# endernewton/tf-faster-rcnn

Hardware: AMD Instinct MI355X
Metric: images/sec (600×1000) ResNet-101 Faster R-CNN at 1/2/4/8 MI355X (higher is better)
Workload: dtype f32 (operands, accumulators, results; GEMMs with Cin, Cout % 128 == 0 form each f32 product from two-piece fp16 operands with an exact power-of-two scale per 128-k block on the fp16 matrix pipe -- 3 MFMAs / product, dropped terms <= 3 * 2^-22, measured error vs float64 below the f32-MFMA kernel's; o

## Files before the change

scratch/h2_conv3.py:

```python
import os, sys
ROOT = os.path.dirname(os.path.dirname(os.path.abspath(__file__)))
sys.path[:0] = [os.path.join(ROOT, "tf-faster-rcnn_amd")]
args = [a for a in sys.argv[1:]]
lib_path, single = None, 0
if "--lib" in args:
    i = args.index("--lib"); lib_path = args[i + 1]; del args[i:i + 2]
if "--single" in args:
    i = args.index("--single"); single = int(args[i + 1]); del args[i:i + 2]
import frcnn_hip
if lib_path:
    frcnn_hip.LIB_PATH = os.path.abspath(lib_path)
import numpy as np, torch
from frcnn_hip import ops
dev = torch.device("cuda:0")
shapes = {
    "b4c3x8":  (1, 117600, 2048, 512, True, True, True, 0),
    "b4c3x8m": (8, 14700, 2048, 512, True, False, False, 49),
    "b3c3x8":  (1, 19152, 1024, 256, True, True, True, 0),
    "b2c3x8":  (1, 75000, 512, 128, True, True, True, 0),
    "b4c3x8p": (1, 117600, 2048, 512, "planes", False, True, 0),
    "b3c3x8p": (1, 19152, 1024, 256, "planes", False, True, 0),
    "b3scx8":  (1, 19152, 1024, 512, False, True, True, 0),
    "w7x8":    (121, 2400, 512, 512, False, True, False, 0),
    "w3x8":    (36, 1280, 256, 256, False, True, False, 0),
    "wrpnx8":  (36, 1280, 512, 1024, False, True, False, 0),
    "b4c1x8":  (1, 117600, 512, 2048, False, False, True, 0),
    "b3c1x8":  (1, 19152, 256, 1024, False, True, False, 0),
    "cal_k128": (1, 117600, 128, 128, "planes", False, True, 0),
    "b4c3x1":  (1, 14700, 2048, 512, True, True, True, 0),
    "b3c3x1":  (1, 2394, 1024, 256, True, True, True, 0),
}
cfgs = [int(c) for c in (args[0] if args else "9,21,12").split(",")]
only = args[1].split(",") if len(args) > 1 else ["b4c3x8", "b4c3x8m", "b3c3x8", "b2c3x8", "w7x8", "w3x8", "b4c1x8", "b3c1x8"]
if not single:
    print("%-8s %-4s %9s %9s %8s %8s  %s" % ("shape", "cfg", "med_us", "min_us", "TFLOP/s", "GB/s", "bits vs cfg %d" % cfgs[0]))
for name in only:
    G, M, N, K, has_res, f32o, planes, mean_rows = shapes[name]
    torch.manual_seed(1)
    x = torch.randn(G * M, K, device=dev).clamp(min=0) * torch.exp(torch.rand(G * M, K, device=dev) * 4 - 2)
    shared_w = mean_rows > 0
    w = torch.randn(1 if shared_w else G, N, K, device=dev) * 0.05
    b = torch.randn(N, device=dev) if (G == 1 or shared_w) else None
    res = torch.randn(G * M, N, device=dev) if has_res else None
    if has_res == "planes":
        res = ops.h2_split(res.clamp(min=0))
    xp, wp = ops.h2_split(x), ops.h2_pack_w(w)
    del x
    outs, outp = {}, {}
    share = G * M * N * 4 > (1 << 29)
    for c in cfgs:
        if mean_rows:
            outs[c] = torch.empty(G * M // mean_rows, N, device=dev)
        else:
            outs[c] = (outs[cfgs[0]] if (share and c != cfgs[0]) else torch.empty(G * M, N, device=dev)) if f32o else None
            outp[c] = (outp[cfgs[0]] if (share and c != cfgs[0]) else ops.H2.empty(G * M, N, dev)) if planes else None

    def run(c):
        if mean_rows:
            return ops.gemm_h2_mean(xp, wp, G, M, N, K, b, res, 1, mean_rows, out=outs[c], cfg=c)
        return ops.gemm_h2(xp, wp, G, M, N, K, b, res, 1, out=outs[c], out_planes=outp.get(c), want_f32=f32o, cfg=c)

    if single:
        for _ in range(single):
            run(cfgs[0])
        torch.cuda.synchronize()
        break
    def digest(c):
        parts = []
        if outs.get(c) is not None:
            parts.append(outs[c].view(torch.int32).to(torch.int64).sum())
            parts.append((outs[c].view(torch.int32).to(torch.int64) * torch.arange(1, outs[c].numel() + 1, device=dev).view(outs[c].shape) % 1000003).sum())
        if outp.get(c) is not None:
            pv = outp[c].planes.view(torch.int16).to(torch.int64)
            parts.append(pv.sum()); parts.append((pv * (torch.arange(pv.numel(), device=dev) % 8191 + 1)).sum())
            parts.append(outp[c].inv.view(torch.int32).to(torch.int64).sum())
        return tuple(int(p) for p in parts)
    digs = {}
    for c in cfgs:
        if outs.get(c) is not None: outs[c].fill_(float("nan"))
        if outp.get(c) is not None: outp[c].planes.zero_(); outp[c].inv.zero_()
        try:
            run(c); torch.cuda.synchronize()
            digs[c] = digest(c)
        except Exception as e:
            digs[c] = "unsupported (%s)" % (str(e)[:60],)
    live = [c for c in cfgs if not isinstance(digs[c], str)]
    times = {c: [] for c in live}
    for r in range(6):
        for c in live:
            e0, e1 = torch.cuda.Event(enable_timing=True), torch.cuda.Event(enable_timing=True)
            e0.record()
            for _ in range(6): run(c)
            e1.record(); torch.cuda.synchronize()
            if r: times[c].append(e0.elapsed_time(e1) * 1000 / 6)
    nbytes = 4.0 * G * M * K + 4.0 * (w.numel()) + G * M * N * 4.0 * ((1 if has_res else 0) + (1 if f32o else 0) + (1 if planes else 0))
    for c in cfgs:
        if c not in live:
            print("%-8s %-4d %s" % (name, c, digs[c]), flush=True)
            continue
        med = float(np.median(times[c]))
        print("%-8s %-4d %9.1f %9.1f %8.1f %8.0f  %s" % (name, c, med, min(times[c]), 2.0 * G * M * N * K / med / 1e6, nbytes / med / 1e3,
                                                       "identical" if digs[c] == digs[cfgs[0]] else "DIFFERENT"), flush=True)
    del outs, outp, xp, res
    torch.cuda.empty_cache()
```

tf-faster-rcnn_amd/csrc/gemm_h2.hip:

```cpp
#include "h2_common.h"
#include <mutex>
#include <type_traits>

typedef float f32x16 __attribute__((ext_vector_type(16)));
typedef _Float16 h8 __attribute__((ext_vector_type(8)));

#define LDS_AS __attribute__((address_space(3)))

struct GemmH2Params {
  const unsigned short* x; const float* x_inv; const unsigned short* w; const float* w_inv;
  const float* bias; const float* res; const unsigned short* resp; const float* resp_inv; float* y; unsigned short* yp; float* y_inv;
  int M, N, K, batch, act, nsteps, mtiles, ntiles;
  long long Mtot;
  int wshare;
  const float* mask;
  float* mean_part; int mean_rows;
};

__device__ __forceinline__ void h2_glds16(unsigned voff, const void* sbase, unsigned lds_base) {
  unsigned keep;
  asm volatile(
      "s_mov_b32 %0, m0\n\t"
      "s_mov_b32 m0, %3\n\t"
      "s_nop 0\n\t"
      "global_load_lds_dwordx4 %1, %2\n\t"
      "s_mov_b32 m0, %0"
      : "=&s"(keep)
      : "v"(voff), "s"(sbase), "s"(lds_base)
      : "memory");
}

__device__ __forceinline__ void h2_glds4(unsigned voff, const void* sbase, unsigned lds_base) {
  unsigned keep;
  asm volatile(
      "s_mov_b32 %0, m0\n\t"
      "s_mov_b32 m0, %3\n\t"
      "s_nop 0\n\t"
      "global_load_lds_dword %1, %2\n\t"
      "s_mov_b32 m0, %0"
      : "=&s"(keep)
      : "v"(voff), "s"(sbase), "s"(lds_base)
      : "memory");
}

__device__ __forceinline__ void h2_glds16c(unsigned voff, const void* sbase, unsigned lds_base) {
  asm volatile(
      "s_mov_b32 m0, %2\n\t"
      "s_nop 0\n\t"
      "global_load_lds_dwordx4 %0, %1"
      :
      : "v"(voff), "s"(sbase), "s"(lds_base)
      : "memory");
}
__device__ __forceinline__ void h2_glds4c(unsigned voff, const void* sbase, unsigned lds_base) {
  asm volatile(
      "s_mov_b32 m0, %2\n\t"
      "s_nop 0\n\t"
      "global_load_lds_dword %0, %1"
      :
      : "v"(voff), "s"(sbase), "s"(lds_base)
      : "memory");
}

template <int N>
__device__ __forceinline__ void h2_wait_vmcnt() {
  asm volatile("s_waitcnt vmcnt(%0)" ::"n"(N) : "memory");
}

enum H2Tune : int {
  H2_SCALES_ONCE = 2,
  H2_PINGPONG = 32,
  H2_MASKED = 128,
  H2_LIGHT_BOUNDARY = 256,
  H2_STORE16 = 512,
  H2_DEFERRED = 1024,
#ifdef FRCNN_ABLATION
  H2_NO_MFMA = 2048,
  H2_NO_FRAG = 4096,
  H2_NO_LOAD = 8192,
#endif
};

template <int BM, int BN, int WM, int WN, int NS, int TUNE>
struct H2Lds {
  static constexpr int NW = (BM / WM) * (BN / WN);
  static constexpr bool PP = (TUNE & H2_PINGPONG) != 0;
  static constexpr int XP = BM * 64, WP = BN * 64;
  static constexpr int S_OFF = 2 * XP + 2 * WP;
  static constexpr int STAGE = S_OFF + (PP ? 0 : 1024);
  static constexpr int RED_OFF = NS * STAGE;
  static constexpr int S2_OFF = RED_OFF + (BN / WN) * BM * 4;
  static constexpr int CB_OFF = S2_OFF + (PP ? NW * 512 : (TUNE & H2_SCALES_ONCE) ? 2048 : 0);
  static constexpr int TOTAL = CB_OFF + ((TUNE & H2_LIGHT_BOUNDARY) ? 2 * 2 * BN * 4 : 0);
};

template <int BM, int BN, int WM, int WN, int NS, int WPE = 2, int TUNE = 0>
__global__ __launch_bounds__((BM / WM) * (BN / WN) * 64) __attribute__((amdgpu_waves_per_eu(WPE))) void k_gemm_h2(const GemmH2Params p) {
  constexpr int NW = (BM / WM) * (BN / WN);
  constexpr int TM = WM / 32, TN = WN / 32;
  constexpr int LA = 2 * BM / 16 / NW;
  constexpr int LB = 2 * BN / 16 / NW;
  constexpr int G = LA + LB;
  constexpr int SL = BM / 64;
  constexpr bool ONCE = (TUNE & H2_SCALES_ONCE) != 0;
  constexpr bool PP = (TUNE & H2_PINGPONG) != 0;
  constexpr bool MASKED = (TUNE & H2_MASKED) != 0;
  constexpr bool LTB = (TUNE & H2_LIGHT_BOUNDARY) != 0;
  constexpr bool W21 = (TUNE & H2_STORE16) != 0;
  constexpr bool DE = (TUNE & H2_DEFERRED) != 0;
  using L = H2Lds<BM, BN, WM, WN, NS, TUNE>;
  constexpr int XP = L::XP, WP = L::WP, S_OFF = L::S_OFF, STAGE = L::STAGE, RED_OFF = L::RED_OFF, S2_OFF = L::S2_OFF, CB_OFF = L::CB_OFF;
  static_assert(!LTB || (!PP && NS == 2 && NW >= 3 && BN % 64 == 0), "light boundary: the two-slot one-barrier-per-slab schedule");
  static_assert(!DE || (LTB && W21 && BN == H2_KB), "deferred epilogue: built on the light boundary's LDS constants and counted waits");
  static_assert(!PP || (NW == 8 && NS == 3 && ONCE && BM == 256 && WM == 64 && BN == 128 && WN == 64),
                "ping-pong geometry: 8 waves as 4 (M) x 2 (N), waves 0-3 = the upper half of the rows");
  static_assert((2 * BM / 16) % NW == 0 && (2 * BN / 16) % NW == 0, "tile/wave mismatch");
  static_assert(BM <= 256 && NS >= 2 && NS <= 4, "stage layout");
  static_assert((NS - 2) * (G + SL) <= 63, "vmcnt range");
  extern __shared__ __attribute__((aligned(16))) char smem[];

  const int tid = threadIdx.x, lane = tid & 63;
  const int wave = __builtin_amdgcn_readfirstlane(tid >> 6);
  const int per = p.mtiles * p.ntiles, T = per * p.batch;
  const int xcd = blockIdx.x & 7, wx = blockIdx.x >> 3, W8 = gridDim.x >> 3;
  const int tq = T / 8, tr = T % 8, tn = tq + (xcd < tr ? 1 : 0);
  const int t_end = (xcd < tr ? xcd * (tq + 1) : tr * (tq + 1) + (xcd - tr) * tq) + tn;
  const int tile0 = t_end - tn + wx;
  if (tile0 >= t_end) return;
  const int my_tiles = (t_end - tile0 + W8 - 1) / W8;
  int left = __builtin_amdgcn_readfirstlane(my_tiles * p.nsteps);

  const int wmi = wave / (BN / WN), wni = wave % (BN / WN);
  const int wm0 = wmi * WM, wn0 = wni * WN;
  const int frow = lane & 31, khalf = lane >> 5;

  const size_t xplane = (size_t)p.Mtot * p.K * 2, wplane = (size_t)p.N * p.K * 2;
  unsigned a_off[LA], b_off[LB], s_off[SL];
  const char* i_xb = nullptr; const char* i_wb = nullptr; const char* i_sb = nullptr;
  int i_tile = tile0, i_step = 0, i_par = 0, c_par = 0;
  int i_g = 0, i_bn0 = 0, i_cpar = 0, c_cpar = 0;
  int pend = 0;
#pragma unroll
  for (int t = 0; t < LB; ++t) {
    const int u = wave * LB + t, plane = u / (BN / 16), row = (u % (BN / 16)) * 16 + (lane >> 2), pos = lane & 3;
    b_off[t] = (unsigned)((size_t)plane * wplane + (size_t)row * p.K * 2 + ((pos ^ ((row >> 2) & 3)) * 16));
  }
  auto tile_coords = [&](int tl, int& g, int& mt, int& nt) {
    g = tl / per;
    const int rem = tl - g * per;
    mt = rem / p.ntiles;
    nt = rem - mt * p.ntiles;
  };
  auto set_tile = [&](int tl) {
    int g, mt, nt;
    tile_coords(tl, g, mt, nt);
    const int bm0 = mt * BM, bn0 = nt * BN;
    const size_t row0 = (size_t)g * p.M + bm0;
    i_g = g; i_bn0 = bn0;
    i_xb = (const char*)p.x + row0 * p.K * 2;
    i_wb = (const char*)p.w + ((size_t)(p.wshare ? 0 : g) * 2 * p.N + bn0) * p.K * 2;
    i_sb = (const char*)(p.x_inv + row0);
#pragma unroll
    for (int t = 0; t < LA; ++t) {
      const int u = wave * LA + t, plane = u / (BM / 16), row = (u % (BM / 16)) * 16 + (lane >> 2), pos = lane & 3;
      const int rr = min(row, p.M - 1 - bm0);
      a_off[t] = (unsigned)((size_t)plane * xplane + (size_t)rr * p.K * 2 + ((pos ^ ((row >> 2) & 3)) * 16));
    }
    const long long last = p.Mtot - 1 - (long long)row0;
#pragma unroll
    for (int j = 0; j < SL; ++j) s_off[j] = (unsigned)(min((long long)((PP ? wm0 : j * 64) + lane), last) * 4);
  };
  const unsigned lds0 = (unsigned)(size_t)(LDS_AS char*)smem;
  auto uniform_ptr = [](const char* q) {
    const unsigned long long v = (unsigned long long)q;
    const unsigned lo = __builtin_amdgcn_readfirstlane((unsigned)v), hi = __builtin_amdgcn_readfirstlane((unsigned)(v >> 32));
    return (const char*)(((unsigned long long)hi << 32) | lo);
  };
  auto issue_one = [&](int buf, int t) {
    const unsigned sb = lds0 + (unsigned)(buf * STAGE);
    if constexpr (PP) {
      if (t < LA) h2_glds16c(a_off[t], uniform_ptr(i_xb), __builtin_amdgcn_readfirstlane(sb + (wave * LA + t) * 1024));
      else if (t < G) h2_glds16c(b_off[t - LA], uniform_ptr(i_wb), __builtin_amdgcn_readfirstlane(sb + 2 * XP + (wave * LB + (t - LA)) * 1024));
      else if (t == G && (i_step & 3) == 0) {
        h2_glds4c(s_off[0], uniform_ptr(i_sb), __builtin_amdgcn_readfirstlane(lds0 + S2_OFF + (wave * 2 + i_par) * 256));
        i_par ^= 1;
      }
      return;
    }
    if (t < LA) h2_glds16(a_off[t], uniform_ptr(i_xb), __builtin_amdgcn_readfirstlane(sb + (wave * LA + t) * 1024));
    else if (t < G) h2_glds16(b_off[t - LA], uniform_ptr(i_wb), __builtin_amdgcn_readfirstlane(sb + 2 * XP + (wave * LB + (t - LA)) * 1024));
    else if (wave == 0) {
      const int j = t - G;
      if (!ONCE) h2_glds4(s_off[j], uniform_ptr(i_sb), __builtin_amdgcn_readfirstlane(sb + S_OFF + j * 256));
      else if ((i_step & 3) == 0) {
        h2_glds4(s_off[j], uniform_ptr(i_sb), __builtin_amdgcn_readfirstlane(lds0 + S2_OFF + i_par * 1024 + j * 256));
        if (j == SL - 1) i_par ^= 1;
      }
    }
  };
  static_assert(!ONCE || NS == 2 || PP, "scales-once needs the uncounted wait of the two-stage ring");
  auto issue_advance = [&]() {
    --left;
    if (++i_step == p.nsteps) {
      i_step = 0; i_tile += W8;
      if (left > 0) set_tile(i_tile);
    } else {
      i_xb += 64; i_wb += 64;
      if ((i_step & 3) == 0) i_sb += (size_t)p.Mtot * 4;
    }
  };

  auto issue_cb = [&]() {
    const unsigned cb = lds0 + CB_OFF + i_cpar * (2 * BN * 4);
    if (wave == 1) {
#pragma unroll
      for (int j = 0; j < BN / 64; ++j)
        h2_glds4((unsigned)(lane * 4), uniform_ptr((const char*)(p.w_inv + (size_t)(p.wshare ? 0 : i_g) * p.N + i_bn0 + j * 64)),
                 __builtin_amdgcn_readfirstlane(cb + j * 256));
    }
    if (wave == 2 && p.bias) {
#pragma unroll
      for (int j = 0; j < BN / 64; ++j)
        h2_glds4((unsigned)(lane * 4), uniform_ptr((const char*)(p.bias + i_bn0 + j * 64)), __builtin_amdgcn_readfirstlane(cb + BN * 4 + j * 256));
    }
    i_cpar ^= 1;
  };
  auto wait_pending = [&](int n) {
    if constexpr (DE) {
      if (n >= 32) {
        if (n >= 48) { if (n >= 56) h2_wait_vmcnt<56>(); else h2_wait_vmcnt<48>(); }
        else { if (n >= 40) h2_wait_vmcnt<40>(); else h2_wait_vmcnt<32>(); }
      } else {
        if (n >= 16) { if (n >= 24) h2_wait_vmcnt<24>(); else h2_wait_vmcnt<16>(); }
        else { if (n >= 8) h2_wait_vmcnt<8>(); else h2_wait_vmcnt<0>(); }
      }
      return;
    }
    if (n >= 63) h2_wait_vmcnt<63>();
    else if (n >= 48) h2_wait_vmcnt<48>();
    else if (n >= 32) h2_wait_vmcnt<32>();
    else if (n >= 16) h2_wait_vmcnt<16>();
    else h2_wait_vmcnt<0>();
  };

  f32x16 tot[TM][TN], tmp[TM][TN];
  const int sw = (frow >> 2) & 3;
  const int x_row = (wm0 + frow) * 64, w_row = 2 * XP + (wn0 + frow) * 64;

#ifdef FRCNN_ABLATION
  constexpr bool NO_MFMA = (TUNE & H2_NO_MFMA) != 0, NO_FRAG = (TUNE & H2_NO_FRAG) != 0, NO_LOAD = (TUNE & H2_NO_LOAD) != 0;
#else
  constexpr bool NO_MFMA = false, NO_FRAG = false, NO_LOAD = false;
#endif
  h8 kxh[NO_FRAG ? TM : 1], kxl[NO_FRAG ? TM : 1], kwh[NO_FRAG ? TN : 1], kwl[NO_FRAG ? TN : 1];
  (void)kxh; (void)kxl; (void)kwh; (void)kwl;
  auto slab_mfma = [&](int cur, auto first_c) {
    constexpr bool FIRST = decltype(first_c)::value;
    const char* sb = smem + cur * STAGE;
#pragma unroll
    for (int t = 0; t < 2; ++t) {
      h8 xh[TM], xl[TM], wh[TN], wl[TN];
      if constexpr (NO_FRAG) {
        if (FIRST && t == 0) {
#pragma unroll
          for (int j = 0; j < TN; ++j) {
            const char* q = sb + w_row + j * 32 * 64 + ((khalf ^ sw) * 16);
            kwh[j] = __builtin_bit_cast(h8, *(const uint4*)(q));
            kwl[j] = __builtin_bit_cast(h8, *(const uint4*)(q + WP));
          }
#pragma unroll
          for (int i = 0; i < TM; ++i) {
            const char* q = sb + x_row + i * 32 * 64 + ((khalf ^ sw) * 16);
            kxh[i] = __builtin_bit_cast(h8, *(const uint4*)(q));
            kxl[i] = __builtin_bit_cast(h8, *(const uint4*)(q + XP));
          }
        }
#pragma unroll
        for (int j = 0; j < TN; ++j) { wh[j] = kwh[j]; wl[j] = kwl[j]; asm volatile("" : "+v"(wh[j]), "+v"(wl[j])); }
#pragma unroll
        for (int i = 0; i < TM; ++i) { xh[i] = kxh[i]; xl[i] = kxl[i]; asm volatile("" : "+v"(xh[i]), "+v"(xl[i])); }
      } else {
#pragma unroll
      for (int j = 0; j < TN; ++j) {
        const char* q = sb + w_row + j * 32 * 64 + (((2 * t + khalf) ^ sw) * 16);
        wh[j] = __builtin_bit_cast(h8, *(const uint4*)(q));
        wl[j] = __builtin_bit_cast(h8, *(const uint4*)(q + WP));
      }
#pragma unroll
      for (int i = 0; i < TM; ++i) {
        const char* q = sb + x_row + i * 32 * 64 + (((2 * t + khalf) ^ sw) * 16);
        xh[i] = __builtin_bit_cast(h8, *(const uint4*)(q));
        xl[i] = __builtin_bit_cast(h8, *(const uint4*)(q + XP));
      }
      }
      if constexpr (NO_MFMA) {
#pragma unroll
        for (int j = 0; j < TN; ++j) asm volatile("" :: "v"(wh[j]), "v"(wl[j]));
#pragma unroll
        for (int i = 0; i < TM; ++i) asm volatile("" :: "v"(xh[i]), "v"(xl[i]));
        if (FIRST && t == 0) {
#pragma unroll
          for (int i = 0; i < TM; ++i)
#pragma unroll
            for (int j = 0; j < TN; ++j)
#pragma unroll
              for (int r = 0; r < 16; ++r) tmp[i][j][r] = 0.f;
        }
        continue;
      }
#pragma unroll
      for (int i = 0; i < TM; ++i)
#pragma unroll
        for (int j = 0; j < TN; ++j) {
          if (FIRST && t == 0) {
            f32x16 z;
#pragma unroll
            for (int r = 0; r < 16; ++r) z[r] = 0.f;
            tmp[i][j] = __builtin_amdgcn_mfma_f32_32x32x16_f16(wh[j], xh[i], z, 0, 0, 0);
          } else {
            tmp[i][j] = __builtin_amdgcn_mfma_f32_32x32x16_f16(wh[j], xh[i], tmp[i][j], 0, 0, 0);
          }
        }
#pragma unroll
      for (int i = 0; i < TM; ++i)
#pragma unroll
        for (int j = 0; j < TN; ++j) {
          tmp[i][j] = __builtin_amdgcn_mfma_f32_32x32x16_f16(wl[j], xh[i], tmp[i][j], 0, 0, 0);
        }
#pragma unroll
      for (int i = 0; i < TM; ++i)
#pragma unroll
        for (int j = 0; j < TN; ++j) {
          tmp[i][j] = __builtin_amdgcn_mfma_f32_32x32x16_f16(wh[j], xl[i], tmp[i][j], 0, 0, 0);
        }
    }
  };

  int c_tile = tile0, c_step = 0, cur = 0, nxt = 0;
  int c_bm0 = 0, c_bn0 = 0, c_g = 0;
  auto set_ctile = [&](int tl) {
    int g, mt, nt;
    tile_coords(tl, g, mt, nt);
    c_bm0 = mt * BM; c_bn0 = nt * BN; c_g = g;
  };
  const float act_lo = p.act == FRCNN_ACT_NONE ? -__builtin_inff() : 0.f;
  const float act_hi = p.act == FRCNN_ACT_RELU6 ? 6.f : __builtin_inff();

  auto rsrc_f = [&](const void* base, long long elems_left, int esize) {
    const long long bytes = elems_left * esize;
    return __builtin_amdgcn_make_buffer_rsrc((void*)base, 0, (int)max(0ll, min(bytes, 0x7fffffffll)), 0x00020000);
  };

  struct TileRef { int bm0, bn0, g, cpar; };
  auto ent_rsrc = [&](const void* base, int g, int esize) {
    const char* b = (const char*)base + (size_t)g * p.M * p.N * esize;
    return __builtin_amdgcn_make_buffer_rsrc((void*)b, 0, p.M * p.N * esize, 0x00020000);
  };
  const int lo4 = (frow * p.N + 4 * khalf) * 4;
  auto lo2_of = [&]() { int v = lo4; asm volatile("" : "+v"(v)); return v >> 1; };
  auto lo2w_of = [&]() { int v = lo4; asm volatile("" : "+v"(v)); return (v >> 1) + 8 * (int)(threadIdx.x >> 5 & 1); };
  auto sub_off = [&](const auto& T, int i, int j) {
    return __builtin_amdgcn_readfirstlane((T.bm0 + wm0 + i * 32) * p.N + T.bn0 + wn0 + j * 32);
  };

  float rri[TM];
  (void)rri;
  auto load_res_raw = [&](int i) {
    typedef unsigned u32x4 __attribute__((ext_vector_type(4)));
    const TileRef C{c_bm0, c_bn0, c_g, c_cpar};
    const bool planes = !p.res && p.resp;
    const auto none = __builtin_amdgcn_make_buffer_rsrc((void*)nullptr, 0, 0, 0x00020000);
    const auto r_even = p.res ? ent_rsrc(p.res, c_g, 4) : planes ? ent_rsrc(p.resp, c_g, 2) : none;
    const auto r_odd = p.res ? r_even : planes ? ent_rsrc(p.resp + (size_t)p.Mtot * p.N, c_g, 2) : none;
    const int step_q = planes ? 0 : 32, step_p = planes ? 32 : 0;
    int base = lo4;
    asm volatile("" : "+v"(base));
    if (planes) base = (base >> 1) + 8 * (int)(threadIdx.x >> 5 & 1);
#pragma unroll
    for (int j = 0; j < TN; ++j) {
      const int vo = base + sub_off(C, i, j) * (planes ? 2 : 4);
#pragma unroll
      for (int q = 0; q < 4; ++q) {
        const u32x4 ld = __builtin_amdgcn_raw_buffer_load_b128((q & 1) ? r_odd : r_even, vo, q * step_q + (q >> 1) * step_p, 0);
        tot[i][j][4 * q + 0] = __uint_as_float(ld[0]); tot[i][j][4 * q + 1] = __uint_as_float(ld[1]);
        tot[i][j][4 * q + 2] = __uint_as_float(ld[2]); tot[i][j][4 * q + 3] = __uint_as_float(ld[3]);
      }
      pend += 4;
    }
    if (p.resp) rri[i] = p.resp_inv[(size_t)(c_bn0 / H2_KB) * p.Mtot + (size_t)c_g * p.M + min(c_bm0 + wm0 + i * 32 + frow, p.M - 1)];
  };
  auto init_tot = [&]() {
    if constexpr (DE) return;
    const size_t row_base = (size_t)c_g * p.M;
    typedef unsigned u32x4 __attribute__((ext_vector_type(4)));
    if (p.res) {
#pragma unroll
      for (int i = 0; i < TM; ++i)
#pragma unroll
        for (int j = 0; j < TN; ++j) {
          const int m0 = c_bm0 + wm0 + i * 32, nc = c_bn0 + wn0 + j * 32;
          const auto rr = rsrc_f(p.res + (long long)(row_base + m0) * p.N + nc, (long long)(p.M - m0) * p.N - nc, 4);
#pragma unroll
          for (int q = 0; q < 4; ++q) {
            const u32x4 ld = __builtin_amdgcn_raw_buffer_load_b128(rr, (frow * p.N + 4 * khalf) * 4 + 32 * q, 0, 0);
            tot[i][j][4 * q + 0] = __uint_as_float(ld[0]); tot[i][j][4 * q + 1] = __uint_as_float(ld[1]);
            tot[i][j][4 * q + 2] = __uint_as_float(ld[2]); tot[i][j][4 * q + 3] = __uint_as_float(ld[3]);
          }
        }
      pend += TM * TN * 4;
    } else if (p.resp) {
      float ri[TM];
#pragma unroll
      for (int i = 0; i < TM; ++i)
        ri[i] = p.resp_inv[(size_t)(c_bn0 / H2_KB) * p.Mtot + row_base + min(c_bm0 + wm0 + i * 32 + frow, p.M - 1)];
      h4 hv[TM][TN][4], lv[TM][TN][4];
#pragma unroll
      for (int i = 0; i < TM; ++i)
#pragma unroll
        for (int j = 0; j < TN; ++j) {
          const int m0 = c_bm0 + wm0 + i * 32, nc = c_bn0 + wn0 + j * 32;
          const long long sbase = (long long)(row_base + m0) * p.N + nc, left_e = (long long)(p.M - m0) * p.N - nc;
          const auto rh = rsrc_f(p.resp + sbase, left_e, 2), rl = rsrc_f(p.resp + (size_t)p.Mtot * p.N + sbase, left_e, 2);
#pragma unroll
          for (int q = 0; q < 4; ++q) {
            const int lo2 = (frow * p.N + 4 * khalf) * 2 + 16 * q;
            hv[i][j][q] = __builtin_bit_cast(h4, __builtin_amdgcn_raw_buffer_load_b64(rh, lo2, 0, 0));
            lv[i][j][q] = __builtin_bit_cast(h4, __builtin_amdgcn_raw_buffer_load_b64(rl, lo2, 0, 0));
          }
        }
#pragma unroll
      for (int i = 0; i < TM; ++i)
#pragma unroll
        for (int j = 0; j < TN; ++j)
#pragma unroll
          for (int q = 0; q < 4; ++q)
#pragma unroll
            for (int e = 0; e < 4; ++e) tot[i][j][4 * q + e] = ((float)hv[i][j][q][e] + (float)lv[i][j][q][e]) * ri[i];
    } else {
#pragma unroll
      for (int i = 0; i < TM; ++i)
#pragma unroll
        for (int j = 0; j < TN; ++j)
#pragma unroll
          for (int r = 0; r < 16; ++r) tot[i][j][r] = 0.f;
    }
    if constexpr (LTB) return;
    float4 wi[TN][4], bv[TN][4];
#pragma unroll
    for (int j = 0; j < TN; ++j)
#pragma unroll
      for (int q = 0; q < 4; ++q)
        wi[j][q] = *(const float4*)(p.w_inv + (size_t)(p.wshare ? 0 : c_g) * p.N + c_bn0 + wn0 + j * 32 + 4 * khalf + 8 * q);
    if (p.bias) {
#pragma unroll
      for (int j = 0; j < TN; ++j)
#pragma unroll
        for (int q = 0; q < 4; ++q) bv[j][q] = *(const float4*)(p.bias + c_bn0 + wn0 + j * 32 + 4 * khalf + 8 * q);
    } else {
#pragma unroll
      for (int j = 0; j < TN; ++j)
#pragma unroll
        for (int q = 0; q < 4; ++q) bv[j][q] = make_float4(0.f, 0.f, 0.f, 0.f);
    }
#pragma unroll
    for (int j = 0; j < TN; ++j)
#pragma unroll
      for (int q = 0; q < 4; ++q) {
        const float s0 = __uint_as_float(0x7f000000u - __float_as_uint(wi[j][q].x)), s1 = __uint_as_float(0x7f000000u - __float_as_uint(wi[j][q].y));
        const float s2 = __uint_as_float(0x7f000000u - __float_as_uint(wi[j][q].z)), s3 = __uint_as_float(0x7f000000u - __float_as_uint(wi[j][q].w));
#pragma unroll
        for (int i = 0; i < TM; ++i) {
          tot[i][j][4 * q + 0] = (tot[i][j][4 * q + 0] + bv[j][q].x) * s0;
          tot[i][j][4 * q + 1] = (tot[i][j][4 * q + 1] + bv[j][q].y) * s1;
          tot[i][j][4 * q + 2] = (tot[i][j][4 * q + 2] + bv[j][q].z) * s2;
          tot[i][j][4 * q + 3] = (tot[i][j][4 * q + 3] + bv[j][q].w) * s3;
        }
      }
  };

  auto ep_scale_act = [&](const TileRef& T) {
#pragma unroll
    for (int j = 0; j < TN; ++j) {
      const int n0 = T.bn0 + wn0 + j * 32 + 4 * khalf;
#pragma unroll
      for (int q = 0; q < 4; ++q) {
        const float4 wi = LTB ? *(const float4*)(smem + CB_OFF + T.cpar * (2 * BN * 4) + (wn0 + j * 32 + 4 * khalf + 8 * q) * 4)
                             : *(const float4*)(p.w_inv + (size_t)(p.wshare ? 0 : T.g) * p.N + n0 + 8 * q);
#pragma unroll
        for (int i = 0; i < TM; ++i) {
          tot[i][j][4 * q + 0] = act_clamp(tot[i][j][4 * q + 0] * wi.x, act_lo, act_hi);
          tot[i][j][4 * q + 1] = act_clamp(tot[i][j][4 * q + 1] * wi.y, act_lo, act_hi);
          tot[i][j][4 * q + 2] = act_clamp(tot[i][j][4 * q + 2] * wi.z, act_lo, act_hi);
          tot[i][j][4 * q + 3] = act_clamp(tot[i][j][4 * q + 3] * wi.w, act_lo, act_hi);
        }
      }
    }
  };
  auto ep_mask = [&](const TileRef& T) {
    if (MASKED && p.mask) {
      const auto rk = ent_rsrc(p.mask, T.g, 4);
#pragma unroll
      for (int i = 0; i < TM; ++i)
#pragma unroll
        for (int j = 0; j < TN; ++j) {
          const int vo = lo4 + sub_off(T, i, j) * 4;
          typedef unsigned u32x4 __attribute__((ext_vector_type(4)));
          u32x4 k[4];
#pragma unroll
          for (int q = 0; q < 4; ++q) k[q] = __builtin_amdgcn_raw_buffer_load_b128(rk, vo + 32 * q, 0, 0);
#pragma unroll
          for (int q = 0; q < 4; ++q)
#pragma unroll
            for (int e = 0; e < 4; ++e) tot[i][j][4 * q + e] = __uint_as_float(k[q][e]) > 0.f ? tot[i][j][4 * q + e] : 0.f;
        }
      pend += TM * TN * 4;
    }
  };
  auto ep_mean = [&](const TileRef& T) {
    const int nblk = (p.M + 31) >> 5;
#pragma unroll
    for (int i = 0; i < TM; ++i) {
      const int mb = T.bm0 + wm0 + i * 32;
      if (mb >= p.M) continue;
      const int m = mb + frow, g0 = mb / p.mean_rows, gid = m / p.mean_rows;
      const bool in_a = m < p.M && gid == g0, in_b = m < p.M && gid == g0 + 1;
      float* dst = p.mean_part + ((size_t)T.g * nblk + (mb >> 5)) * 2 * p.N;
#pragma unroll
      for (int j = 0; j < TN; ++j) {
        const int n0 = T.bn0 + wn0 + j * 32 + 4 * khalf;
#pragma unroll
        for (int q = 0; q < 4; ++q) {
          float a[4], b[4];
#pragma unroll
          for (int e = 0; e < 4; ++e) {
            const float v = tot[i][j][4 * q + e];
            a[e] = in_a ? v : 0.f;
            b[e] = in_b ? v : 0.f;
          }
#pragma unroll
          for (int o = 1; o < 32; o <<= 1)
#pragma unroll
            for (int e = 0; e < 4; ++e) {
              a[e] += __shfl_xor(a[e], o, 64);
              b[e] += __shfl_xor(b[e], o, 64);
            }
          if (frow == 0) {
            *(float4*)(dst + n0 + 8 * q) = make_float4(a[0], a[1], a[2], a[3]);
            *(float4*)(dst + p.N + n0 + 8 * q) = make_float4(b[0], b[1], b[2], b[3]);
          }
          pend += 2;
        }
      }
    }
  };
  auto ep_store_f32 = [&](const TileRef& T, int i) {
    if (!p.y) return;
    const auto ry = ent_rsrc(p.y, T.g, 4);
#pragma unroll
    for (int j = 0; j < TN; ++j) {
      const int lo = lo4 + sub_off(T, i, j) * 4;
#pragma unroll
      for (int q = 0; q < 4; ++q) {
        typedef unsigned u32x4 __attribute__((ext_vector_type(4)));
        u32x4 o;
        o[0] = __float_as_uint(tot[i][j][4 * q + 0]); o[1] = __float_as_uint(tot[i][j][4 * q + 1]);
        o[2] = __float_as_uint(tot[i][j][4 * q + 2]); o[3] = __float_as_uint(tot[i][j][4 * q + 3]);
        __builtin_amdgcn_raw_buffer_store_b128(o, ry, lo + 32 * q, 0, 0);
      }
      pend += 4;
      if constexpr (DE) __builtin_amdgcn_sched_barrier(0);
    }
  };
  auto ep_rowmax_write = [&](float (&mx)[TM]) {
    float* red = (float*)(smem + RED_OFF);
#pragma unroll
    for (int i = 0; i < TM; ++i) {
      float m = 0.f;
#pragma unroll
      for (int j = 0; j < TN; ++j)
#pragma unroll
        for (int r = 0; r < 16; ++r) m = fmaxf(m, fabsf(tot[i][j][r]));
      m = fmaxf(m, __shfl_xor(m, 32, 64));
      mx[i] = m;
      if (BN / WN > 1 && khalf == 0) red[wni * BM + wm0 + i * 32 + frow] = m;
    }
  };
  auto ep_rowmax_merge = [&](float (&mx)[TM]) {
    const float* red = (const float*)(smem + RED_OFF);
#pragma unroll
    for (int i = 0; i < TM; ++i)
#pragma unroll
      for (int o = 0; o < BN / WN; ++o) mx[i] = fmaxf(mx[i], red[o * BM + wm0 + i * 32 + frow]);
  };
  auto ep_store_planes = [&](const TileRef& T, int i, float mxi) {
    const size_t row_base = (size_t)T.g * p.M;
    const size_t yplane = (size_t)p.Mtot * p.N;
    float scale, inv;
    h2_block_scale(mxi, scale, inv);
    const int m0 = T.bm0 + wm0 + i * 32;
    if (wni == 0 && khalf == 0 && m0 + frow < p.M)
      p.y_inv[(size_t)(T.bn0 / H2_KB) * p.Mtot + row_base + m0 + frow] = inv;
    const auto rh = ent_rsrc(p.yp, T.g, 2), rl = ent_rsrc(p.yp + yplane, T.g, 2);
#pragma unroll
    for (int j = 0; j < TN; ++j) {
      const int so = sub_off(T, i, j) * 2;
      typedef unsigned u32x2 __attribute__((ext_vector_type(2)));
      if constexpr (W21) {
        const int lo = lo2w_of() + so;
#pragma unroll
        for (int pq = 0; pq < 2; ++pq) {
          h4 ha, la, hb, lb;
          h2_split4(make_float4(tot[i][j][8 * pq + 0], tot[i][j][8 * pq + 1], tot[i][j][8 * pq + 2], tot[i][j][8 * pq + 3]), scale, ha, la);
          h2_split4(make_float4(tot[i][j][8 * pq + 4], tot[i][j][8 * pq + 5], tot[i][j][8 * pq + 6], tot[i][j][8 * pq + 7]), scale, hb, lb);
          const u32x2 uha = __builtin_bit_cast(u32x2, ha), uhb = __builtin_bit_cast(u32x2, hb);
          const u32x2 ula = __builtin_bit_cast(u32x2, la), ulb = __builtin_bit_cast(u32x2, lb);
          typedef unsigned u32x4 __attribute__((ext_vector_type(4)));
          const auto h0 = __builtin_amdgcn_permlane32_swap(uha[0], uhb[0], false, false), h1 = __builtin_amdgcn_permlane32_swap(uha[1], uhb[1], false, false);
          const auto l0 = __builtin_amdgcn_permlane32_swap(ula[0], ulb[0], false, false), l1 = __builtin_amdgcn_permlane32_swap(ula[1], ulb[1], false, false);
          __builtin_amdgcn_raw_buffer_store_b128(u32x4{h0[0], h1[0], h0[1], h1[1]}, rh, lo + 32 * pq, 0, 0);
          __builtin_amdgcn_raw_buffer_store_b128(u32x4{l0[0], l1[0], l0[1], l1[1]}, rl, lo + 32 * pq, 0, 0);
        }
        pend += 4;
        if constexpr (DE) __builtin_amdgcn_sched_barrier(0);
      } else {
        const int lo = lo2_of() + so;
#pragma unroll
        for (int q = 0; q < 4; ++q) {
          h4 hh, ll;
          h2_split4(make_float4(tot[i][j][4 * q + 0], tot[i][j][4 * q + 1], tot[i][j][4 * q + 2], tot[i][j][4 * q + 3]), scale, hh, ll);
          __builtin_amdgcn_raw_buffer_store_b64(__builtin_bit_cast(u32x2, hh), rh, lo + 16 * q, 0, 0);
          __builtin_amdgcn_raw_buffer_store_b64(__builtin_bit_cast(u32x2, ll), rl, lo + 16 * q, 0, 0);
        }
        pend += 8;
      }
    }
  };

  auto epilogue = [&]() {
    const TileRef T{c_bm0, c_bn0, c_g, c_cpar};
    ep_scale_act(T);
    ep_mask(T);
    if (p.mean_part) {
      ep_mean(T);
      c_cpar ^= 1;
      return;
    }
#pragma unroll
    for (int i = 0; i < TM; ++i) ep_store_f32(T, i);
    if (p.yp) {
      float mx[TM];
      ep_rowmax_write(mx);
      if (BN / WN > 1) {
        asm volatile("s_waitcnt lgkmcnt(0)" ::: "memory");
        __builtin_amdgcn_s_barrier();
        ep_rowmax_merge(mx);
      }
#pragma unroll
      for (int i = 0; i < TM; ++i) ep_store_planes(T, i, mx[i]);
      if (BN / WN > 1) {
        asm volatile("s_waitcnt lgkmcnt(0)" ::: "memory");
        __builtin_amdgcn_s_barrier();
      }
    }
    c_cpar ^= 1;
  };

  constexpr int HALF = (TM + 1) / 2;
  bool have_prev = false;
  TileRef P{0, 0, 0, 0};
  float dmx[TM];
  (void)dmx;
  auto de_piece = [&](auto pos_c) {
    constexpr int POS = decltype(pos_c)::value;
    if constexpr (POS == 0) {
      if (have_prev) {
        ep_scale_act(P);
        ep_mask(P);
        if (p.yp) ep_rowmax_write(dmx);
      }
    } else if constexpr (POS == 1 || POS == 2) {
      constexpr int I0 = POS == 1 ? 0 : HALF, I1 = POS == 1 ? HALF : TM;
      if (have_prev) {
        if (POS == 1 && p.yp && BN / WN > 1) ep_rowmax_merge(dmx);
#pragma unroll
        for (int i = I0; i < I1; ++i) {
          ep_store_f32(P, i);
          if (p.yp) ep_store_planes(P, i, dmx[i]);
        }
      }
#pragma unroll
      for (int i = I0; i < I1; ++i) load_res_raw(i);
    }
  };

  auto slab = [&](auto pos_c, bool fold, bool first_block) {
    constexpr int POS = decltype(pos_c)::value;
    const std::integral_constant<bool, POS == 0> first_c{};
    if constexpr (DE) asm volatile("s_waitcnt lgkmcnt(0)" ::: "memory");
    if constexpr (LTB) {
      wait_pending(pend);
    } else if (left >= 1) {
      if (wave == 0) h2_wait_vmcnt<(NS - 2) * (G + SL)>(); else h2_wait_vmcnt<(NS - 2) * G>();
    } else {
      h2_wait_vmcnt<0>();
    }
    __builtin_amdgcn_s_barrier();
    const bool more = left > 0;
    if (more) {
#pragma unroll
      for (int t = 0; t < (NO_LOAD ? 0 : G + SL); ++t) issue_one(nxt, t);
      if constexpr (LTB) {
        if (i_step == 0) issue_cb();
        pend = 0;
      }
    }
    if constexpr (DE) {
      __builtin_amdgcn_sched_barrier(0);
      if (first_block) de_piece(pos_c);
      __builtin_amdgcn_sched_barrier(0);
    }
    float ainv[TM];
    if (fold) {
      const int soff = ONCE ? S2_OFF + c_par * 1024 : cur * STAGE + S_OFF;
#pragma unroll
      for (int i = 0; i < TM; ++i) ainv[i] = *(const float*)(smem + soff + (wm0 + i * 32 + frow) * 4);
      c_par ^= 1;
    }
    slab_mfma(cur, first_c);
    if (more) {
      issue_advance();
      nxt = nxt + 1 == NS ? 0 : nxt + 1;
    }
    if (fold) {
      if (LTB && first_block) {
        const float* cbp = (const float*)(smem + CB_OFF + c_cpar * (2 * BN * 4));
        if (DE && !p.res && p.resp) {
          typedef unsigned u32x2 __attribute__((ext_vector_type(2)));
#pragma unroll
          for (int i = 0; i < TM; ++i)
#pragma unroll
            for (int j = 0; j < TN; ++j)
#pragma unroll
              for (int pq = 0; pq < 2; ++pq) {
                unsigned w[8];
#pragma unroll
                for (int e = 0; e < 8; ++e) w[e] = __float_as_uint(tot[i][j][8 * pq + e]);
                const auto h0 = __builtin_amdgcn_permlane32_swap(w[0], w[2], false, false), h1 = __builtin_amdgcn_permlane32_swap(w[1], w[3], false, false);
                const auto l0 = __builtin_amdgcn_permlane32_swap(w[4], w[6], false, false), l1 = __builtin_amdgcn_permlane32_swap(w[5], w[7], false, false);
                const h4 ha = __builtin_bit_cast(h4, u32x2{h0[0], h1[0]}), hb = __builtin_bit_cast(h4, u32x2{h0[1], h1[1]});
                const h4 la = __builtin_bit_cast(h4, u32x2{l0[0], l1[0]}), lb = __builtin_bit_cast(h4, u32x2{l0[1], l1[1]});
#pragma unroll
                for (int e = 0; e < 4; ++e) {
                  tot[i][j][8 * pq + e] = ((float)ha[e] + (float)la[e]) * rri[i];
                  tot[i][j][8 * pq + 4 + e] = ((float)hb[e] + (float)lb[e]) * rri[i];
                }
              }
        }
#pragma unroll
        for (int j = 0; j < TN; ++j)
#pragma unroll
          for (int q = 0; q < 4; ++q) {
            const float4 wi = *(const float4*)(cbp + wn0 + j * 32 + 4 * khalf + 8 * q);
            const float4 bv = p.bias ? *(const float4*)(cbp + BN + wn0 + j * 32 + 4 * khalf + 8 * q) : make_float4(0.f, 0.f, 0.f, 0.f);
            const float s0 = __uint_as_float(0x7f000000u - __float_as_uint(wi.x)), s1 = __uint_as_float(0x7f000000u - __float_as_uint(wi.y));
            const float s2 = __uint_as_float(0x7f000000u - __float_as_uint(wi.z)), s3 = __uint_as_float(0x7f000000u - __float_as_uint(wi.w));
#pragma unroll
            for (int i = 0; i < TM; ++i) {
              tot[i][j][4 * q + 0] = __builtin_fmaf(tmp[i][j][4 * q + 0], ainv[i], (tot[i][j][4 * q + 0] + bv.x) * s0);
              tot[i][j][4 * q + 1] = __builtin_fmaf(tmp[i][j][4 * q + 1], ainv[i], (tot[i][j][4 * q + 1] + bv.y) * s1);
              tot[i][j][4 * q + 2] = __builtin_fmaf(tmp[i][j][4 * q + 2], ainv[i], (tot[i][j][4 * q + 2] + bv.z) * s2);
              tot[i][j][4 * q + 3] = __builtin_fmaf(tmp[i][j][4 * q + 3], ainv[i], (tot[i][j][4 * q + 3] + bv.w) * s3);
            }
          }
      } else {
#pragma unroll
        for (int i = 0; i < TM; ++i)
#pragma unroll
          for (int j = 0; j < TN; ++j)
#pragma unroll
            for (int r = 0; r < 16; ++r) tot[i][j][r] = __builtin_fmaf(tmp[i][j][r], ainv[i], tot[i][j][r]);
      }
    }
    cur = cur + 1 == NS ? 0 : cur + 1;
  };

  set_tile(i_tile);
  set_ctile(c_tile);
  if constexpr (PP) {
    const int grp = wave >> 2;
    h8 fxh[2][TM], fxl[2][TM], fwh[2][TN], fwl[2][TN];
    auto seg_barrier = [&]() {
      __builtin_amdgcn_sched_barrier(0);
      __builtin_amdgcn_s_barrier();
      __builtin_amdgcn_sched_barrier(0);
    };
    auto fold = [&]() {
      float ainv[TM];
#pragma unroll
      for (int i = 0; i < TM; ++i) ainv[i] = *(const float*)(smem + S2_OFF + (wave * 2 + c_par) * 256 + (i * 32 + frow) * 4);
      c_par ^= 1;
#pragma unroll
      for (int i = 0; i < TM; ++i)
#pragma unroll
        for (int j = 0; j < TN; ++j)
#pragma unroll
          for (int r = 0; r < 16; ++r) tot[i][j][r] = __builtin_fmaf(tmp[i][j][r], ainv[i], tot[i][j][r]);
    };
    auto pp_mem = [&](auto pos_c, bool fold_prev) -> bool {
      constexpr int POS = decltype(pos_c)::value;
      const char* sb = smem + cur * STAGE;
#pragma unroll
      for (int t = 0; t < 2; ++t) {
#pragma unroll
        for (int j = 0; j < TN; ++j) {
          const char* q = sb + w_row + j * 32 * 64 + (((2 * t + khalf) ^ sw) * 16);
          fwh[t][j] = __builtin_bit_cast(h8, *(const uint4*)(q));
          fwl[t][j] = __builtin_bit_cast(h8, *(const uint4*)(q + WP));
        }
#pragma unroll
        for (int i = 0; i < TM; ++i) {
          const char* q = sb + x_row + i * 32 * 64 + (((2 * t + khalf) ^ sw) * 16);
          fxh[t][i] = __builtin_bit_cast(h8, *(const uint4*)(q));
          fxl[t][i] = __builtin_bit_cast(h8, *(const uint4*)(q + XP));
        }
      }
      const bool more = left > 0;
      if (more) {
#pragma unroll
        for (int t = 0; t <= G; ++t) issue_one(nxt, t);
        issue_advance();
        nxt = nxt + 1 == NS ? 0 : nxt + 1;
      }
      if (fold_prev) fold();
      if (grp == 1) {
        if (more) h2_wait_vmcnt<(POS == 2 ? G + 1 : G)>(); else h2_wait_vmcnt<0>();
      }
      asm volatile("s_waitcnt lgkmcnt(0)" ::: "memory");
      seg_barrier();
      return more;
    };
    auto pp_mfma = [&](auto pos_c, bool issued) {
      constexpr int POS = decltype(pos_c)::value;
      __builtin_amdgcn_s_setprio(1);
#pragma unroll
      for (int t = 0; t < 2; ++t) {
#pragma unroll
        for (int i = 0; i < TM; ++i)
#pragma unroll
          for (int j = 0; j < TN; ++j) {
            if (POS == 0 && t == 0) {
              f32x16 z;
#pragma unroll
              for (int r = 0; r < 16; ++r) z[r] = 0.f;
              tmp[i][j] = __builtin_amdgcn_mfma_f32_32x32x16_f16(fwh[t][j], fxh[t][i], z, 0, 0, 0);
            } else {
              tmp[i][j] = __builtin_amdgcn_mfma_f32_32x32x16_f16(fwh[t][j], fxh[t][i], tmp[i][j], 0, 0, 0);
            }
          }
#pragma unroll
        for (int i = 0; i < TM; ++i)
#pragma unroll
          for (int j = 0; j < TN; ++j) tmp[i][j] = __builtin_amdgcn_mfma_f32_32x32x16_f16(fwl[t][j], fxh[t][i], tmp[i][j], 0, 0, 0);
#pragma unroll
        for (int i = 0; i < TM; ++i)
#pragma unroll
          for (int j = 0; j < TN; ++j) tmp[i][j] = __builtin_amdgcn_mfma_f32_32x32x16_f16(fwh[t][j], fxl[t][i], tmp[i][j], 0, 0, 0);
      }
      __builtin_amdgcn_s_setprio(0);
      if (grp == 0) {
        if (issued) h2_wait_vmcnt<(POS == 2 ? G + 1 : G)>(); else h2_wait_vmcnt<0>();
      }
      cur = cur + 1 == NS ? 0 : cur + 1;
      seg_barrier();
    };
    bool two = false;
#pragma unroll
    for (int s2 = 0; s2 < 2; ++s2) {
      if (left > 0) {
#pragma unroll
        for (int t = 0; t <= G; ++t) issue_one(nxt, t);
        issue_advance();
        nxt = nxt + 1 == NS ? 0 : nxt + 1;
        two = s2 == 1;
      }
    }
    if (two) h2_wait_vmcnt<G>(); else h2_wait_vmcnt<0>();
    seg_barrier();
    if (grp == 1) seg_barrier();
    const int nkb = p.nsteps >> 2;
    for (int tl = 0; tl < my_tiles; ++tl) {
      init_tot();
      for (int kb = 0; kb < nkb; ++kb) {
        bool is;
        is = pp_mem(std::integral_constant<int, 0>{}, kb > 0); pp_mfma(std::integral_constant<int, 0>{}, is);
        is = pp_mem(std::integral_constant<int, 1>{}, false);  pp_mfma(std::integral_constant<int, 1>{}, is);
        is = pp_mem(std::integral_constant<int, 2>{}, false);  pp_mfma(std::integral_constant<int, 2>{}, is);
        is = pp_mem(std::integral_constant<int, 3>{}, false);  pp_mfma(std::integral_constant<int, 3>{}, is);
      }
      fold();
      epilogue();
      c_tile += W8;
      if (tl + 1 < my_tiles) set_ctile(c_tile);
    }
    if (grp == 0) seg_barrier();
    h2_wait_vmcnt<0>();
    return;
  }
#pragma unroll
  for (int s = 0; s < NS - 1; ++s) {
// ... 267 lines not shown
```

tf-faster-rcnn_amd/csrc/h2_common.h:

```cpp
#pragma once
#include "common.h"

typedef _Float16 h4 __attribute__((ext_vector_type(4)));
typedef _Float16 h2v __attribute__((ext_vector_type(2)));

#define H2_KB 128

__device__ __forceinline__ void h2_block_scale_bits(unsigned mx_bits, float& scale, float& inv) {
  int ex = (int)((mx_bits >> 23) & 0xffu);
  ex = ex < 15 ? 15 : ex;
  scale = __uint_as_float((unsigned)(268 - ex) << 23);
  inv = __uint_as_float((unsigned)(ex - 14) << 23);
}
__device__ __forceinline__ void h2_block_scale(float mx, float& scale, float& inv) { h2_block_scale_bits(__float_as_uint(mx), scale, inv); }

__device__ __forceinline__ void h2_split1(float v, float scale, _Float16& h, _Float16& l) {
  const float vs = v * scale;
  h = (_Float16)vs;
  l = (_Float16)(vs - (float)h);
}

__device__ __forceinline__ unsigned h2_abs_bits(float v) { return __float_as_uint(v) & 0x7fffffffu; }
__device__ __forceinline__ unsigned h2_abs_bits4(float4 v) {
  return max(max(h2_abs_bits(v.x), h2_abs_bits(v.y)), max(h2_abs_bits(v.z), h2_abs_bits(v.w)));
}

template <int CTRL>
__device__ __forceinline__ unsigned h2_dpp(unsigned v) { return __builtin_amdgcn_update_dpp(v, v, CTRL, 0xf, 0xf, false); }
__device__ __forceinline__ unsigned h2_max16(unsigned v) {
  v = max(v, h2_dpp<0xB1>(v));
  v = max(v, h2_dpp<0x4E>(v));
  v = max(v, h2_dpp<0x141>(v));
  v = max(v, h2_dpp<0x140>(v));
  return v;
}
__device__ __forceinline__ unsigned h2_max32(unsigned v) {
  v = h2_max16(v);
  const auto r = __builtin_amdgcn_permlane16_swap(v, v, false, false);
  return max(r[0], r[1]);
}
__device__ __forceinline__ unsigned h2_max64(unsigned v) {
  v = h2_max32(v);
  const auto r = __builtin_amdgcn_permlane32_swap(v, v, false, false);
  return max(r[0], r[1]);
}

typedef float f32x4v __attribute__((ext_vector_type(4)));
typedef float f32x2v __attribute__((ext_vector_type(2)));

__device__ __forceinline__ void h2_split4(float4 v, float scale, h4& hh, h4& ll) {
  const f32x4v vs = f32x4v{v.x, v.y, v.z, v.w} * scale;
  hh = __builtin_convertvector(vs, h4);
  ll = __builtin_convertvector(vs - __builtin_convertvector(hh, f32x4v), h4);
}
__device__ __forceinline__ void h2_split2(float2 v, float scale, h2v& hh, h2v& ll) {
  const f32x2v vs = f32x2v{v.x, v.y} * scale;
  hh = __builtin_convertvector(vs, h2v);
  ll = __builtin_convertvector(vs - __builtin_convertvector(hh, f32x2v), h2v);
}

template <int NR>
__device__ __forceinline__ void h2_emit_rows32(const float4* v, const size_t* e, float* const* inv_slot, unsigned valid,
                                               unsigned short* __restrict__ planes, size_t plane, int l32) {
  unsigned mx = 0;
#pragma unroll
  for (int n = 0; n < NR; ++n)
    if ((valid >> n) & 1u) mx = max(mx, h2_abs_bits4(v[n]));
  mx = h2_max32(mx);
  float scale, inv;
  h2_block_scale_bits(mx, scale, inv);
#pragma unroll
  for (int n = 0; n < NR; ++n) {
    if (!((valid >> n) & 1u)) continue;
    h4 hh, ll;
    h2_split4(v[n], scale, hh, ll);
    *(h4*)(planes + e[n]) = hh;
    *(h4*)(planes + plane + e[n]) = ll;
    if (l32 == 0) *inv_slot[n] = inv;
  }
}

template <int NR>
__device__ __forceinline__ void h2_emit_rows64(const float2* v, const size_t* e, float* const* inv_slot, unsigned valid,
                                               unsigned short* __restrict__ planes, size_t plane, int l64) {
  unsigned mx = 0;
#pragma unroll
  for (int n = 0; n < NR; ++n)
    if ((valid >> n) & 1u) mx = max(mx, max(h2_abs_bits(v[n].x), h2_abs_bits(v[n].y)));
  mx = h2_max64(mx);
  float scale, inv;
  h2_block_scale_bits(mx, scale, inv);
#pragma unroll
  for (int n = 0; n < NR; ++n) {
    if (!((valid >> n) & 1u)) continue;
    h2v hh, ll;
    h2_split2(v[n], scale, hh, ll);
    *(h2v*)(planes + e[n]) = hh;
    *(h2v*)(planes + plane + e[n]) = ll;
    if (l64 == 0) *inv_slot[n] = inv;
  }
}
```

Baseline: 536.4.

## Stage residual-plane inverse scales through LDS and use DPP sums in mean epilogue

Residual-plane inverse scales are now prefetched into LDS by wave 3 alongside the bias/scale slab, so the fold reads them from LDS instead of issuing per-row scalar global loads. This also enables the plane-residual fold on the non-deferred light-boundary path. The mean epilogue's 32-lane reductions switch from shfl_xor chains to DPP/permlane sums, and the second group's reduction is skipped when a 32-row block does not cross a group boundary. The light-boundary static assert is tightened (NW>=4, BM<=128), and a new benchmark shape is added.

```diff
diff --git a/scratch/h2_conv3.py b/scratch/h2_conv3.py
--- a/scratch/h2_conv3.py
+++ b/scratch/h2_conv3.py
@@ -16,6 +16,7 @@
 shapes = {
     "b4c3x8":  (1, 117600, 2048, 512, True, True, True, 0),
     "b4c3x8m": (8, 14700, 2048, 512, True, False, False, 49),
+    "b4c3x8pm": (8, 14700, 2048, 512, "planes", False, False, 49),
     "b3c3x8":  (1, 19152, 1024, 256, True, True, True, 0),
     "b2c3x8":  (1, 75000, 512, 128, True, True, True, 0),
     "b4c3x8p": (1, 117600, 2048, 512, "planes", False, True, 0),
diff --git a/tf-faster-rcnn_amd/csrc/gemm_h2.hip b/tf-faster-rcnn_amd/csrc/gemm_h2.hip
--- a/tf-faster-rcnn_amd/csrc/gemm_h2.hip
+++ b/tf-faster-rcnn_amd/csrc/gemm_h2.hip
@@ -92,6 +92,7 @@
   static constexpr int S2_OFF = RED_OFF + (BN / WN) * BM * 4;
   static constexpr int CB_OFF = S2_OFF + (PP ? NW * 512 : (TUNE & H2_SCALES_ONCE) ? 2048 : 0);
   static constexpr int TOTAL = CB_OFF + ((TUNE & H2_LIGHT_BOUNDARY) ? 2 * 2 * BN * 4 : 0);
+  static constexpr int RI_OFF = S_OFF + 512;
 };
 
 template <int BM, int BN, int WM, int WN, int NS, int WPE = 2, int TUNE = 0>
@@ -109,8 +110,8 @@
   constexpr bool W21 = (TUNE & H2_STORE16) != 0;
   constexpr bool DE = (TUNE & H2_DEFERRED) != 0;
   using L = H2Lds<BM, BN, WM, WN, NS, TUNE>;
-  constexpr int XP = L::XP, WP = L::WP, S_OFF = L::S_OFF, STAGE = L::STAGE, RED_OFF = L::RED_OFF, S2_OFF = L::S2_OFF, CB_OFF = L::CB_OFF;
-  static_assert(!LTB || (!PP && NS == 2 && NW >= 3 && BN % 64 == 0), "light boundary: the two-slot one-barrier-per-slab schedule");
+  constexpr int XP = L::XP, WP = L::WP, S_OFF = L::S_OFF, STAGE = L::STAGE, RED_OFF = L::RED_OFF, S2_OFF = L::S2_OFF, CB_OFF = L::CB_OFF, RI_OFF = L::RI_OFF;
+  static_assert(!LTB || (!PP && NS == 2 && NW >= 4 && BN % 64 == 0 && BM <= 128), "light boundary: the two-slot one-barrier-per-slab schedule");
   static_assert(!DE || (LTB && W21 && BN == H2_KB), "deferred epilogue: built on the light boundary's LDS constants and counted waits");
   static_assert(!PP || (NW == 8 && NS == 3 && ONCE && BM == 256 && WM == 64 && BN == 128 && WN == 64),
                 "ping-pong geometry: 8 waves as 4 (M) x 2 (N), waves 0-3 = the upper half of the rows");
@@ -138,7 +139,7 @@
   unsigned a_off[LA], b_off[LB], s_off[SL];
   const char* i_xb = nullptr; const char* i_wb = nullptr; const char* i_sb = nullptr;
   int i_tile = tile0, i_step = 0, i_par = 0, c_par = 0;
-  int i_g = 0, i_bn0 = 0, i_cpar = 0, c_cpar = 0;
+  int i_g = 0, i_bm0 = 0, i_bn0 = 0, i_cpar = 0, c_cpar = 0;
   int pend = 0;
 #pragma unroll
   for (int t = 0; t < LB; ++t) {
@@ -156,7 +157,7 @@
     tile_coords(tl, g, mt, nt);
     const int bm0 = mt * BM, bn0 = nt * BN;
     const size_t row0 = (size_t)g * p.M + bm0;
-    i_g = g; i_bn0 = bn0;
+    i_g = g; i_bm0 = bm0; i_bn0 = bn0;
     i_xb = (const char*)p.x + row0 * p.K * 2;
     i_wb = (const char*)p.w + ((size_t)(p.wshare ? 0 : g) * 2 * p.N + bn0) * p.K * 2;
     i_sb = (const char*)(p.x_inv + row0);
@@ -222,6 +223,12 @@
 #pragma unroll
       for (int j = 0; j < BN / 64; ++j)
         h2_glds4((unsigned)(lane * 4), uniform_ptr((const char*)(p.bias + i_bn0 + j * 64)), __builtin_amdgcn_readfirstlane(cb + BN * 4 + j * 256));
+    }
+    if (wave == 3 && p.resp) {
+      const char* rb = (const char*)(p.resp_inv + (size_t)(i_bn0 / H2_KB) * p.Mtot + (size_t)i_g * p.M + i_bm0);
+#pragma unroll
+      for (int j = 0; j < SL; ++j)
+        h2_glds4((unsigned)(min(j * 64 + lane, p.M - 1 - i_bm0) * 4), uniform_ptr(rb), __builtin_amdgcn_readfirstlane(lds0 + i_cpar * STAGE + RI_OFF + j * 256));
     }
     i_cpar ^= 1;
   };
@@ -363,8 +370,6 @@
     return __builtin_amdgcn_readfirstlane((T.bm0 + wm0 + i * 32) * p.N + T.bn0 + wn0 + j * 32);
   };
 
-  float rri[TM];
-  (void)rri;
   auto load_res_raw = [&](int i) {
     typedef unsigned u32x4 __attribute__((ext_vector_type(4)));
     const TileRef C{c_bm0, c_bn0, c_g, c_cpar};
@@ -387,10 +392,23 @@
       }
       pend += 4;
     }
-    if (p.resp) rri[i] = p.resp_inv[(size_t)(c_bn0 / H2_KB) * p.Mtot + (size_t)c_g * p.M + min(c_bm0 + wm0 + i * 32 + frow, p.M - 1)];
   };
   auto init_tot = [&]() {
     if constexpr (DE) return;
+    if constexpr (LTB) {
+      if (p.res || p.resp) {
+#pragma unroll
+        for (int i = 0; i < TM; ++i) load_res_raw(i);
+      } else {
+#pragma unroll
+        for (int i = 0; i < TM; ++i)
+#pragma unroll
+          for (int j = 0; j < TN; ++j)
+#pragma unroll
+            for (int r = 0; r < 16; ++r) tot[i][j][r] = 0.f;
+      }
+      return;
+    }
     const size_t row_base = (size_t)c_g * p.M;
     typedef unsigned u32x4 __attribute__((ext_vector_type(4)));
     if (p.res) {
@@ -444,7 +462,6 @@
 #pragma unroll
           for (int r = 0; r < 16; ++r) tot[i][j][r] = 0.f;
     }
-    if constexpr (LTB) return;
     float4 wi[TN][4], bv[TN][4];
 #pragma unroll
     for (int j = 0; j < TN; ++j)
@@ -516,39 +533,30 @@
       pend += TM * TN * 4;
     }
   };
-  auto ep_mean = [&](const TileRef& T) {
+  auto ep_mean = [&](const TileRef& T, int i) {
+    const int mb = T.bm0 + wm0 + i * 32;
+    if (mb >= p.M) return;
     const int nblk = (p.M + 31) >> 5;
-#pragma unroll
-    for (int i = 0; i < TM; ++i) {
-      const int mb = T.bm0 + wm0 + i * 32;
-      if (mb >= p.M) continue;
-      const int m = mb + frow, g0 = mb / p.mean_rows, gid = m / p.mean_rows;
-      const bool in_a = m < p.M && gid == g0, in_b = m < p.M && gid == g0 + 1;
-      float* dst = p.mean_part + ((size_t)T.g * nblk + (mb >> 5)) * 2 * p.N;
-#pragma unroll
-      for (int j = 0; j < TN; ++j) {
-        const int n0 = T.bn0 + wn0 + j * 32 + 4 * khalf;
-#pragma unroll
-        for (int q = 0; q < 4; ++q) {
-          float a[4], b[4];
-#pragma unroll
-          for (int e = 0; e < 4; ++e) {
-            const float v = tot[i][j][4 * q + e];
-            a[e] = in_a ? v : 0.f;
-            b[e] = in_b ? v : 0.f;
-          }
-#pragma unroll
-          for (int o = 1; o < 32; o <<= 1)
-#pragma unroll
-            for (int e = 0; e < 4; ++e) {
-              a[e] += __shfl_xor(a[e], o, 64);
-              b[e] += __shfl_xor(b[e], o, 64);
-            }
-          if (frow == 0) {
-            *(float4*)(dst + n0 + 8 * q) = make_float4(a[0], a[1], a[2], a[3]);
-            *(float4*)(dst + p.N + n0 + 8 * q) = make_float4(b[0], b[1], b[2], b[3]);
-          }
-          pend += 2;
+    const int m = mb + frow, g0 = mb / p.mean_rows, gid = m / p.mean_rows;
+    const bool in_a = m < p.M && gid == g0, in_b = m < p.M && gid == g0 + 1;
+    const bool two = mb - g0 * p.mean_rows + 31 >= p.mean_rows;
+    float* dst = p.mean_part + ((size_t)T.g * nblk + (mb >> 5)) * 2 * p.N;
+#pragma unroll
+    for (int j = 0; j < TN; ++j) {
+      const int n0 = T.bn0 + wn0 + j * 32 + 4 * khalf;
+#pragma unroll
+      for (int q = 0; q < 4; ++q) {
+        float a[4];
+#pragma unroll
+        for (int e = 0; e < 4; ++e) a[e] = h2_sum32(in_a ? tot[i][j][4 * q + e] : 0.f);
+        if (frow == 0) *(float4*)(dst + n0 + 8 * q) = make_float4(a[0], a[1], a[2], a[3]);
+        ++pend;
+        if (two) {
+          float b[4];
+#pragma unroll
+          for (int e = 0; e < 4; ++e) b[e] = h2_sum32(in_b ? tot[i][j][4 * q + e] : 0.f);
+          if (frow == 0) *(float4*)(dst + p.N + n0 + 8 * q) = make_float4(b[0], b[1], b[2], b[3]);
+          ++pend;
         }
       }
     }
@@ -641,7 +649,8 @@
     ep_scale_act(T);
     ep_mask(T);
     if (p.mean_part) {
-      ep_mean(T);
+#pragma unroll
+      for (int i = 0; i < TM; ++i) ep_mean(T, i);
       c_cpar ^= 1;
       return;
     }
@@ -734,10 +743,11 @@
     if (fold) {
       if (LTB && first_block) {
         const float* cbp = (const float*)(smem + CB_OFF + c_cpar * (2 * BN * 4));
-        if (DE && !p.res && p.resp) {
+        if (!p.res && p.resp) {
           typedef unsigned u32x2 __attribute__((ext_vector_type(2)));
 #pragma unroll
-          for (int i = 0; i < TM; ++i)
+          for (int i = 0; i < TM; ++i) {
+            const float rri = *(const float*)(smem + c_cpar * STAGE + RI_OFF + (wm0 + i * 32 + frow) * 4);
 #pragma unroll
             for (int j = 0; j < TN; ++j)
 #pragma unroll
@@ -751,10 +761,11 @@
                 const h4 la = __builtin_bit_cast(h4, u32x2{l0[0], l1[0]}), lb = __builtin_bit_cast(h4, u32x2{l0[1], l1[1]});
 #pragma unroll
                 for (int e = 0; e < 4; ++e) {
-                  tot[i][j][8 * pq + e] = ((float)ha[e] + (float)la[e]) * rri[i];
-                  tot[i][j][8 * pq + 4 + e] = ((float)hb[e] + (float)lb[e]) * rri[i];
+                  tot[i][j][8 * pq + e] = ((float)ha[e] + (float)la[e]) * rri;
+                  tot[i][j][8 * pq + 4 + e] = ((float)hb[e] + (float)lb[e]) * rri;
                 }
               }
+          }
         }
 #pragma unroll
         for (int j = 0; j < TN; ++j)
diff --git a/tf-faster-rcnn_amd/csrc/h2_common.h b/tf-faster-rcnn_amd/csrc/h2_common.h
--- a/tf-faster-rcnn_amd/csrc/h2_common.h
+++ b/tf-faster-rcnn_amd/csrc/h2_common.h
@@ -43,6 +43,19 @@
   v = h2_max32(v);
   const auto r = __builtin_amdgcn_permlane32_swap(v, v, false, false);
   return max(r[0], r[1]);
+}
+
+template <int CTRL>
+__device__ __forceinline__ float h2_dpp_f32(float v) {
+  return __uint_as_float(__builtin_amdgcn_update_dpp(0u, __float_as_uint(v), CTRL, 0xf, 0xf, false));
+}
+__device__ __forceinline__ float h2_sum32(float v) {
+  v += h2_dpp_f32<0xB1>(v);
+  v += h2_dpp_f32<0x4E>(v);
+  v += h2_dpp_f32<0x141>(v);
+  v += h2_dpp_f32<0x140>(v);
+  const auto r = __builtin_amdgcn_permlane16_swap(__float_as_uint(v), __float_as_uint(v), false, false);
+  return __uint_as_float(r[0]) + __uint_as_float(r[1]);
 }
 
 typedef float f32x4v __attribute__((ext_vector_type(4)));
```

After: 545.8, median of 6. 1.02x the previous value.
